# blepping/ComfyUI-sonar

Measured on AMD Instinct MI355X. Metric: noise-latents/sec (SDXL 4x128x128), higher is better.
Workload: dtype f32

## Files before the change

### comfyui-sonar_amd/csrc/plan.hip

```cpp
#include <math.h>
#include <string.h>

#include <memory>
#include <type_traits>
#include <utility>
#include <vector>

#include "common.h"

namespace sonar {
namespace {

template <typename T>
inline T word_to(uint64_t w) {
    if constexpr (std::is_pointer_v<T>) {
        return reinterpret_cast<T>(static_cast<uintptr_t>(w));
    } else if constexpr (std::is_same_v<T, float>) {
        const uint32_t lo = (uint32_t)w;
        float f;
        memcpy(&f, &lo, sizeof f);
        return f;
    } else if constexpr (std::is_same_v<T, double>) {
        double d;
        memcpy(&d, &w, sizeof d);
// ... 42 lines not shown
    SONAR_REPLAYABLE(sonar_philox_normal_chain_f32),
    SONAR_REPLAYABLE(sonar_perlin_lattice_f32),
    SONAR_REPLAYABLE(sonar_perlin_generate_f32),
    SONAR_REPLAYABLE(sonar_perlin_generate_acc_f32),
    SONAR_REPLAYABLE(sonar_perlin_generate_chain_f32),
    SONAR_REPLAYABLE(sonar_perlin_noise_f32),
    SONAR_REPLAYABLE(sonar_perlin_noise_ahead_f32),
    SONAR_REPLAYABLE(sonar_pyramid_generate_f32),
    SONAR_REPLAYABLE(sonar_pyramid_generate_acc_f32),
    SONAR_REPLAYABLE(sonar_pyramid_generate_acc_ahead_f32),
    SONAR_REPLAYABLE(sonar_pyramid_noise_f32),
    SONAR_REPLAYABLE(sonar_pyramid_noise_ahead_f32),
    SONAR_REPLAYABLE(sonar_power_noise_f32),
    SONAR_REPLAYABLE(sonar_power_block_f32),
    SONAR_REPLAYABLE(sonar_power_noise_ahead_f32),
    SONAR_REPLAYABLE(sonar_power_irfft2_f32),
    SONAR_REPLAYABLE(sonar_spectral_filter_f32),
    SONAR_REPLAYABLE(sonar_channel_mix_f32),
    SONAR_REPLAYABLE(sonar_std_scale_f32),
    SONAR_REPLAYABLE(sonar_powerlaw_f32),
    SONAR_REPLAYABLE(sonar_mul_table_f32),
    SONAR_REPLAYABLE(sonar_stats_finalize),
    SONAR_REPLAYABLE(sonar_scale_noise_rows_f32),
    SONAR_REPLAYABLE(sonar_blend_f32),
    SONAR_REPLAYABLE(sonar_blend_tensor_f32),
    SONAR_REPLAYABLE(sonar_scalar_op_f32),
    SONAR_REPLAYABLE(sonar_rowstats_f32),
    SONAR_REPLAYABLE(sonar_row_affine_f32),
    SONAR_REPLAYABLE(sonar_amax_mid_f32),
    SONAR_REPLAYABLE(sonar_div_mid_f32),
// ... 212 lines not shown
```

### comfyui-sonar_amd/csrc/power_fft.hip

```cpp
#include "power_core.h"

namespace sonar {

template <int H, int W>
constexpr int plane_min_waves() {
    return (H * W >= 32768 || (H == 256 && W == 64) || (H == 64 && W == 256) || (H == 64 && W == 32)) ? 2 : 4;
}

template <int H, int W, int SRC, bool STATS, bool NORM>
__global__ void __launch_bounds__((plane_threads<H, W>()), (plane_min_waves<H, W>())) power_irfft2_kernel(const float* __restrict__ z,
                                                                       const float* __restrict__ filter, float* out,
                                                                       int64_t planes, uint64_t seed, uint64_t stream_id,
                                                                       int64_t plane_offset, int group, int split, double* partials,
                                                                       NormArgs na, StatsAhead sa) {
    kernarg_touch_for(z, filter, out, planes, seed, stream_id, plane_offset, group, split, partials, na, sa);
    using C = PlaneCfg<H, W>;
    constexpr int NT = plane_threads<H, W>();
    constexpr int M = C::M, S = C::S;
    constexpr int RN1 = C::RN1, RN2 = C::RN2;
    constexpr bool FAST = (W == 128) && (H == 128 || H == 64) && (NT == 512);
    constexpr int CN1 = FAST ? H / 8 : C::CN1, CN2 = FAST ? 8 : C::CN2;
    __shared__ c32 A[C::kLdsComplex];
    c32* const T0 = A + H * S;
    c32* const TM = T0 + H;
// ... 1021 lines not shown
            }
            partials_next[2 * slot] = ss;
            partials_next[2 * slot + 1] = qq;
        }
    }
};

template <int IT0, int IT1, int N>
__device__ __forceinline__ void pin_chunk(c32 (&v)[N]) {
#pragma unroll
    for (int it = IT0; it < IT1; ++it) {
        asm volatile("" : "+v"(v[it].x), "+v"(v[it].y), "+v"(v[it + N / 2].x), "+v"(v[it + N / 2].y));
    }
}

template <int H, int W, bool STATS, bool NORM>
__global__ void __launch_bounds__(1024) power_pipe_kernel(const float* __restrict__ filter, float* out, int64_t planes, uint64_t seed,
                                                          uint64_t stream_id, int64_t plane_offset, int group, int split, double* partials,
                                                          NormArgs na, uint64_t next_stream, double* partials_next) {
    kernarg_touch_for(filter, out, planes, seed, stream_id, plane_offset, group, split, partials, na, next_stream, partials_next);
    using C = PlaneCfg<H, W>;
    constexpr int NT = 512, NALL = 1024;
    static_assert(plane_threads<H, W>() == NT && W == 128 && H == 128, "one 8-wave team per plane, slot = one radix-16 column item");
    constexpr int M = C::M, S = C::S, Wh = M + 1, RN1 = C::RN1, RN2 = C::RN2, CN1 = H / 8, CN2 = 8, ITER = draw_iters<H, W>();
    constexpr int LM = draw_shift<W>();
    constexpr int E0 = kPipeChunks[0], E1 = E0 + kPipeChunks[1];
    static_assert(E1 <= ITER && ITER == CN1 / 2, "chunks of whole pair iterations");
    constexpr int BUF = H * S;
    __shared__ c32 PLANES[2 * BUF];
    __shared__ c32 EDGE[3 * H];
    __shared__ uint4 SEED_RT[NT];
    static_assert(sizeof(uint4) * NT >= sizeof(c32) * 2 * H * kAheadMaxGroup, "edge columns of a look-ahead unit fit the seed area");
    __shared__ double sred[2 * NT / 64];
    __shared__ double red[2 * NALL / 64];
    __shared__ NormDecision shd;
    const int wv_all = __builtin_amdgcn_readfirstlane((int)threadIdx.x >> 6);
    const bool drawer = wv_all >= NT / 64;
    const int tid = threadIdx.x & (NT - 1), lane = threadIdx.x & 63, wv = wv_all & (NT / 64 - 1);
    const int64_t nunits = split ? planes : planes / group;
    const int64_t group0 = plane_offset / group;
    const int per_unit = split ? 1 : group;
    const int64_t my_units = (int64_t)blockIdx.x < nunits ? (nunits - blockIdx.x + gridDim.x - 1) / gridDim.x : 0;
    const int n = (int)(my_units * per_unit);
    const bool ahead = partials_next != nullptr && nunits <= 2 * (int64_t)gridDim.x;
    const float scale = 1.0f / sqrtf((float)H * (float)W);
    float nm = scale, nc = 0.0f;
    static_assert(!NORM || kNPart == NALL, "one partial pair per thread");
    [[maybe_unused]] double pre_s = 0.0, pre_q = 0.0;
    if constexpr (NORM) {
        pre_s = na.partials[2 * threadIdx.x];
        pre_q = na.partials[2 * threadIdx.x + 1];
    }
    auto leave_wave_sums = [&]() {
        if constexpr (NORM) {
            const double ws = wave_sum(pre_s), wq = wave_sum(pre_q);
            if (lane == 0) {
                red[wv_all] = ws;
                red[NALL / 64 + wv_all] = wq;
            }
        }
    };
    auto decide_in_wave0 = [&]() {
        if constexpr (NORM) {
            if (wv_all == 0) {
                double ss = 0.0, qq = 0.0;
#pragma unroll
                for (int i = 0; i < NALL / 64; ++i) {
                    ss += red[i];
                    qq += red[NALL / 64 + i];
                }
                const NormDecision dec = decision_from_totals(ss, qq, na.n_total, na.thr_sd);
                if (lane == 0) shd = dec;
            }
        }
    };
    auto pick_up_decision = [&]() {
        if constexpr (NORM) {
            const NormDecision dec = shd;
            const float g = (dec.do_div ? 1.0f / dec.stdv : 1.0f) * na.factor;
            nm = scale * g;
            nc = dec.do_sub ? dec.mean * g : 0.0f;
        }
    };
    double s = 0.0, q = 0.0;
    if (drawer) {
        __builtin_amdgcn_s_setprio(kPipePrioDraw);
        const c32* const Q = EDGE + 2 * H;
        SpectrumRng rng;
        float wa[ITER], wb[ITER];
        bool neg = false;
#pragma unroll
        for (int it = 0; it < ITER; ++it) {
            const int p = tid + it * NT, pos = (p >> LM) * Wh + 1 + (p & (M - 1));
            const float fa = filter[pos], fb = filter[pos + (H / 2) * Wh];
            wa[it] = filter_weight(fa);
            wb[it] = filter_weight(fb);
            neg = neg || fa < 0.0f || fb < 0.0f;
        }
        const bool wave_neg = __builtin_amdgcn_ballot_w64(neg) != 0;
        c32 ctw[CN1];
#pragma unroll
        for (int k1 = 0; k1 < CN1; ++k1) ctw[k1] = c_tw256[((wv * k1) * (256 / H)) & 255];
        const int col = (lane + 1) & (M - 1);
        int64_t unit = blockIdx.x;
        int gp = 0;
        for (int j = 0; j < n; ++j) {
            c32* const A = PLANES + (j & 1) * BUF;
            c32 v[CN1];
            SONAR_PIPE_STAMP(0);
            if (gp == 0) {
                const GroupWalk gw(unit, group, split);
                if (j == per_unit) {
                    const uint4 rt = SEED_RT[tid];
                    rng.R = Mwc{rt.x, rt.y};
                    rng.T = Mwc{rt.z, rt.w};
                } else {
                    rng = spectrum_seed<true>(seed, stream_id, group0 + gw.grp, tid, false);
                }
                for (int i = 0; i < gw.first; ++i) skip_plane<H, W, true, false>(rng, tid);
            }
            draw_chunk_regs<H, W, 0, E0>(rng, v, wa, wb);
            if (wave_neg) draw_chunk_signs<H, W, 0, E0>(filter, tid, v);
            pin_chunk<0, E0>(v);
            SONAR_PIPE_STAMP(1);
            __syncthreads();
            draw_chunk_regs<H, W, E0, E1>(rng, v, wa, wb);
            if (wave_neg) draw_chunk_signs<H, W, E0, E1>(filter, tid, v);
            pin_chunk<E0, E1>(v);
            SONAR_PIPE_STAMP(2);
            __syncthreads();
            draw_chunk_regs<H, W, E1, ITER>(rng, v, wa, wb);
            if (wave_neg) draw_chunk_signs<H, W, E1, ITER>(filter, tid, v);
// ... 4 lines not shown
            idft<CN1>(v);
#pragma unroll
            for (int k1 = 1; k1 < CN1; ++k1) v[k1] = cmul(v[k1], ctw[k1]);
#pragma unroll
            for (int k1 = 0; k1 < CN1; ++k1) A[(CN2 * k1 + wv) * S + col] = v[k1];
            if (++gp == per_unit) {
                gp = 0;
                unit += gridDim.x;
            }
            if (j == 0) leave_wave_sums();
            SONAR_PIPE_STAMP(3);
            __syncthreads();
        }
        [[maybe_unused]] const int j = n;
        SONAR_PIPE_STAMP(0);
        if (ahead && my_units == 2) {
            TeamStats<H, W> ts;
            c32* const edge = reinterpret_cast<c32*>(SEED_RT);
            const GroupWalk gw((int64_t)blockIdx.x + gridDim.x, group, split);
            ts.begin(filter, seed, next_stream, plane_offset, group, gw, tid, edge, wa, wb);
            ts.radii(0, kAheadSplitA, tid);
            SONAR_PIPE_STAMP(1);
            __syncthreads();
            ts.radii(kAheadSplitA, kAheadSplitB, tid);
            SONAR_PIPE_STAMP(2);
            __syncthreads();
            ts.radii(kAheadSplitB, 4, tid);
            ts.products();
            ts.edges_and_wave_sums(edge, tid, sred);
            SONAR_PIPE_STAMP(3);
            __syncthreads();
// ... 7 lines not shown
        }
    } else {
        __builtin_amdgcn_s_setprio(kPipePrioFft);
        int64_t unit = blockIdx.x;
        int gp = 0;
        c32* const T0 = EDGE;
        c32* const TM = EDGE + H;
        c32* const Q = EDGE + 2 * H;
        const float f0 = tid < H ? filter[tid * Wh] : 0.0f, fm = tid < H ? filter[tid * Wh + M] : 0.0f;
        Mwc rngE{0, 1}, rngE2{0, 1};
        int64_t eunit = blockIdx.x;
        int egp = 0;
        auto draw_edges = [&](int je) {
            if (tid < H && je < n) {
                if (egp == 0) {
                    const GroupWalk gw(eunit, group, split);
                    rngE = je == per_unit ? rngE2 : spectrum_seed<false>(seed, stream_id, group0 + gw.grp, tid, true).E;
                    for (int i = 0; i < 3 * gw.first; ++i) rngE.next();
                }
                const uint32_t r0 = rngE.next();
                const uint32_t rm = rngE.next();
                const uint32_t t = rngE.next();
                T0[tid] = drawn_elem(r0, angle_lo(t), f0);
                TM[tid] = drawn_elem(rm, angle_hi(t), fm);
                if (++egp == per_unit) {
                    egp = 0;
                    eunit += gridDim.x;
                }
            }
        };
        auto pack_edges = [&](int je) {
            if (tid >= NT - H && je < n) {
                const int ky = tid - (NT - H), kn = (H - ky) & (H - 1);
                const c32 a = T0[ky], an = T0[kn], b = TM[ky], bn = TM[kn];
                Q[ky] = make_float2(0.5f * (a.x + an.x) - 0.5f * (b.y - bn.y), 0.5f * (a.y - an.y) + 0.5f * (b.x + bn.x));
            }
        };
        if (n > per_unit) {
            const GroupWalk gw(unit + gridDim.x, group, split);
            const SpectrumRng g2 = spectrum_rng<H, true>(seed, stream_id, group0 + gw.grp, tid);
            SEED_RT[tid] = make_uint4(g2.R.x, g2.R.c, g2.T.x, g2.T.c);
            rngE2 = g2.E;
        }
        [[maybe_unused]] const int j = 0;
        SONAR_PIPE_STAMP(0);
        auto exchange = [] { __syncthreads(); };
        if (ahead && my_units >= 1) {
            TeamStats<H, W> ts;
            c32* const edge = PLANES + BUF;
            const GroupWalk gw(unit, group, split);
            if (blockIdx.x == 0)
                for (int64_t slot = nunits + tid; slot < kNPart; slot += NT) {
                    partials_next[2 * slot] = 0.0;
                    partials_next[2 * slot + 1] = 0.0;
                }
            __builtin_amdgcn_s_setprio(kAheadPrio);
            draw_edges(0);
            ts.begin(filter, seed, next_stream, plane_offset, group, gw, tid, edge);
            ts.radii(0, kAheadSplitC, tid);
            SONAR_PIPE_STAMP(1);
            exchange();
            pack_edges(0);
// ... 15 lines not shown
            pack_edges(0);
            SONAR_PIPE_STAMP(2);
            exchange();
            leave_wave_sums();
            SONAR_PIPE_STAMP(3);
            __syncthreads();
        }
        for (int j = 1; j <= n; ++j) {
            constexpr int NW = 8;
            const bool work = j >= 1;
            c32* const X = PLANES + ((j + 1) & 1) * BUF;
            c32* const Y = PLANES + (j & 1) * BUF;
            SONAR_PIPE_STAMP(0);
            if (work) pipe_col_b<H, W, NW>(X, Y, wv, lane);
            draw_edges(j);
            if (j == 1) decide_in_wave0();
            SONAR_PIPE_STAMP(1);
            exchange();
            if (work) pipe_row_a<H, W, NW>(Y, X, wv, lane);
            pack_edges(j);
            SONAR_PIPE_STAMP(2);
            exchange();
            if (work) {
                if (j == 1) pick_up_decision();
                const GroupWalk gw(unit, group, split);
                float* const oplane = out + (gw.grp * group + gw.first + gp) * (int64_t)H * W;
                pipe_row_b<H, W, NW, STATS, NORM>(X, oplane, wv, lane, scale, nm, nc, s, q);
                if (++gp == per_unit) {
                    gp = 0;
                    unit += gridDim.x;
                }
            }
            SONAR_PIPE_STAMP(3);
            __syncthreads();
        }
    }
    if (ahead) {
        __syncthreads();
        if (drawer && my_units == 2) TeamStats<H, W>::store(sred, tid, partials_next, (int64_t)blockIdx.x + gridDim.x);
    }
    if constexpr (STATS) write_partial<NALL>(s, q, partials, red);
}

template <int H, int W>
__device__ __forceinline__ void power_stats_body(const float* __restrict__ filter, int64_t planes, uint64_t seed, uint64_t stream_id,
                                                 int64_t plane_offset, int group, int split, double* partials, int64_t bid, int64_t nb,
                                                 c32 (*EDGE)[2][H] , double* red) {
    constexpr int NT = plane_threads<H, W>(), M = W / 2, Wh = M + 1;
    constexpr int NB = kStatsBatch;
    const int tid = threadIdx.x;
    double s = 0.0, q = 0.0;
    auto edge_terms = [&](int p) {
        float edge = 0.0f;
        for (int ky = tid; ky < H; ky += NT) {
            const int kn = (H - ky) & (H - 1);
            const c32 a = EDGE[p][0][ky], an = EDGE[p][0][kn], b = EDGE[p][1][ky], bn = EDGE[p][1][kn];
// ... 352 lines not shown
    SONAR_REQUIRE(filter && out && partials && planes >= 0 && H > 0 && W > 0 && plane_offset >= 0, SONAR_ERR_ARG,
                  "sonar_power_noise_ahead_f32: bad argument");
    SONAR_REQUIRE((reinterpret_cast<uintptr_t>(out) & 7u) == 0 && partials_next != partials, SONAR_ERR_ARG,
                  "sonar_power_noise_ahead_f32: misaligned buffer, or the same workspace for both calls' statistics");
    SONAR_REQUIRE(sonar_power_noise_ahead_ok(planes, H, W, rng_group), SONAR_ERR_UNSUPPORTED,
                  "sonar_power_noise_ahead_f32: no look-ahead for %lld planes of %lld x %lld (ask sonar_power_noise_ahead_ok first)", (long long)planes,
                  (long long)H, (long long)W);
    Ahead ah;
    ah.have_stats = have_stats != 0;
    ah.next_stream = next_stream_id;
    ah.next = partials_next;
    return power_dispatch(1, nullptr, filter, out, planes, H, W, seed, stream_id, plane_offset, rng_group, partials,
                          NormArgs{partials, planes * H * W, factor, threshold_std_devs}, (hipStream_t)stream, ah);
}

extern "C" int sonar_spectral_filter_f32(const float* x, const float* filter, float* out, int64_t planes, int64_t H, int64_t W,
                                         double* partials, void* stream) {
    SONAR_REQUIRE(x && filter && out && x != out && planes >= 0 && H > 0 && W > 0, SONAR_ERR_ARG,
                  "sonar_spectral_filter_f32: bad argument (in-place not supported)");
    SONAR_REQUIRE((reinterpret_cast<uintptr_t>(out) & 7u) == 0 && (reinterpret_cast<uintptr_t>(x) & 7u) == 0, SONAR_ERR_ARG,
                  "sonar_spectral_filter_f32: misaligned buffer");
    if (planes == 0) return SONAR_OK;
    return power_dispatch(3, x, filter, out, planes, H, W, 0, 0, 0, 1, partials, NormArgs{nullptr, 0, 1.0f, 0.0f}, (hipStream_t)stream);
}

extern "C" int sonar_rfft2_f32(const float* x, float* z_out, int64_t planes, int64_t H, int64_t W, void* stream) {
    SONAR_REQUIRE(x && z_out && planes >= 0 && H > 0 && W > 0, SONAR_ERR_ARG, "sonar_rfft2_f32: bad argument");
    SONAR_REQUIRE((reinterpret_cast<uintptr_t>(z_out) & 7u) == 0 && (reinterpret_cast<uintptr_t>(x) & 7u) == 0, SONAR_ERR_ARG,
                  "sonar_rfft2_f32: misaligned buffer");
    if (planes == 0) return SONAR_OK;
// ... 27 lines not shown
```

### comfyui-sonar_amd/hip_lib.py

```python
from __future__ import annotations

import ctypes as C
import math
import os
import threading as _threading
import weakref
from typing import Optional, Sequence

import torch

_HERE = os.path.dirname(os.path.abspath(__file__))
LIB_PATH = os.path.join(_HERE, "libsonar_hip.so")

BLEND_IDS = {"lerp": 0, "inject": 1, "subtract_b": 2}
MODE_IDS = {"CLASSIC": 0, "NEW": 1, "DENOISED": 2}
INIT_IDS = {"NONE": 0, "SAMPLE": 1, "SAMPLE_NORM": 2}
RESAMPLE_IDS = {"bilinear": 0, "nearest-exact": 1, "area": 2, "adaptive_avg_pool2d": 2, "nearest": 3, "bicubic": 4, "bicubic_aligned": 5,
                "bilinear_aligned": 6}
UPSCALE_MODES = ("bilinear", "nearest-exact", "area", "adaptive_avg_pool2d", "nearest", "bicubic")
PYRAMID_FUSED_MODES = ("bilinear", "nearest-exact", "area", "adaptive_avg_pool2d")
DWT_MODE_IDS = {"zero": 0, "symmetric": 1, "reflect": 2, "periodization": 3, "periodic": 4, "constant": 5, "replicate": 5}
NPART = 1024
BROWNIAN_MAX_TERMS = 96
ERR_ARG, ERR_UNSUPPORTED, ERR_HIP = -1, -2, -3
# ... 93 lines not shown
    "sonar_perlin_noise_ahead_ok": (_I, [_I64, _I64, _I64]),
    "sonar_perlin_noise_ahead_f32": (_I, [_P, _P, _I64, _I64, _F, _U64, _U64, _I64, _F, _F, _P, _I, _U64, _P, _P, _P, _I64, _I64, _I64, _I64, _I, _U64, _P]),
    "sonar_resample_acc_f32": (_I, [_P, _P, _I64, _I64, _I64, _I64, _I64, _F, _I, _I, _P, _P]),
    "sonar_pyramid_generate_f32": (_I, [_P, _I64, _I64, _I64, _I64, C.POINTER(_P), _PI64, _PI64, _PF, _I, _U64, _U64, _I64, _P, _P]),
    "sonar_pyramid_route": (_I, [_I64, _I64, _I64, _PI64, _PI64, _I, _I64]),
    "sonar_pyramid_noise_f32": (_I, [_P, _I64, _I64, _I64, _I64, C.POINTER(_P), _PI64, _PI64, _PF, _I, _U64, _U64, _I64, _F, _F, _P, _P]),
    "sonar_pyramid_noise_ahead_f32": (_I, [_P, _I64, _I64, _I64, _I64, _PI64, _PI64, _PF, _I, _U64, _U64, _I64, _F, _F, _P, _I, _U64, _I64, _PI64, _PI64, _PF, _P,
                                           _P]),
    "sonar_levels_sampled_f32": (_I, [_P, _I64, _I64, _I64, _I, _PI64, _PI64, _PF, _PF, _I, _U64, _U64, _I64, _I, _P]),
    "sonar_level_normal_f32": (_I, [_P, _I64, _I64, _I64, _F, _U64, _U64, _I64, _P]),
    "sonar_power_noise_f32": (_I, [_P, _P, _I64, _I64, _I64, _U64, _U64, _I64, _I, _F, _F, _P, _P]),
    "sonar_power_noise_ahead_ok": (_I, [_I64, _I64, _I64, _I]),
    "sonar_power_pipeline": (_I, [_I]),
    "sonar_wcfg_hi_storage": (_I, [_I]),
    "sonar_power_noise_ahead_f32": (_I, [_P, _P, _I64, _I64, _I64, _U64, _U64, _I64, _I, _F, _F, _P, _I, _U64, _P, _P]),
    "sonar_power_spectrum_f32": (_I, [_P, _I64, _I64, _I64, _U64, _U64, _I64, _I, _P]),
    "sonar_power_irfft2_f32": (_I, [_P, _P, _P, _I64, _I64, _I64, _U64, _U64, _I64, _I, _P, _P]),
    "sonar_spectral_filter_f32": (_I, [_P, _P, _P, _I64, _I64, _I64, _P, _P]),
    "sonar_std_scale_f32": (_I, [_P, _I64, _F, _P, _I64, _I64, _P]),
    "sonar_channel_mix_f32": (_I, [_P, _P, _P, _I64, _I64, _I64, _P, _P]),
    "sonar_dwt_out_len": (_I64, [_I64, _I64, _I]),
    "sonar_dwt2_ws_bytes": (_I64, [_I64, _I64, _I64, _I, _I, _I, _I]),
    "sonar_dwt2_fwd_f32": (_I, [_P, _P, _P, _I64, _I64, _I64, _PD, _PD, _I, _I, _P, _P]),
    "sonar_dwt2_fwd_f64": (_I, [_P, _P, _P, _I64, _I64, _I64, _PD, _PD, _I, _I, _P, _P]),
    "sonar_dwt2_inv_f32": (_I, [_P, _I64, _I64, _P, _P, _I64, _I64, _I64, _I64, _I64, _PD, _PD, _I, _I, _P, _P]),
    "sonar_dwt2_inv_f64": (_I, [_P, _I64, _I64, _P, _P, _I64, _I64, _I64, _I64, _I64, _PD, _PD, _I, _I, _P, _P]),
    "sonar_sq_acc_f32": (_I, [_P, _P, _F, _I, _I64, _P]),
    "sonar_studentt_f32": (_I, [_P, _P, _F, _F, _F, _I64, _P]),
    "sonar_abs_quantile_rows_f32": (_I, [_P, _I64, _I64, _I64, _F, _P, _P]),
    "sonar_clamp_signpow_rows_f32": (_I, [_P, _I64, _I64, _P, _F, _F, _P]),
# ... 992 lines not shown
    if kind in (3, 4):
        if z is None:
            white = philox_normal(tuple(shape), filt.device, seed, stream_id, plane_offset * H * W)
            return _direct_spectral_filter(white, filt, partials)
        return _direct_inverse(z, filt, out, 1.0 / math.sqrt(H * W), partials)
    _check(
        load().sonar_power_irfft2_f32(zp, _dev(filt, "filter"), _dev(out, "out"), planes, H, W, seed & (2**64 - 1), stream_id, plane_offset,
                                      rng_group_for(shape), _opt(partials, "partials", torch.float64), _stream()),
        "sonar_power_irfft2_f32",
    )
    return out


class PowerLookahead:

    __slots__ = ("key", "partials", "last_stream", "last_delta", "step", "hits", "misses")

    def __init__(self):
        self.key = None
        self.partials = None
        self.last_stream = None
        self.last_delta = None
        self.step = 1
        self.hits = 0
        self.misses = 0


def power_noise(filt: torch.Tensor, shape, *, seed: int, stream_id: int, plane_offset: int, factor: float,
                threshold_std_devs: float = 2.5, lookahead: Optional[PowerLookahead] = None) -> torch.Tensor:
    H, W = shape[-2:]
    out = torch.empty(shape, dtype=torch.float32, device=filt.device)
    planes = out.numel() // (H * W)
    kind = power_plane_kind(H, W)
    if kind == 4:
        return _power_block(1, filt, out, seed, stream_id, plane_offset, partials=new_partials(filt.device), factor=factor,
                            threshold_std_devs=threshold_std_devs)
    if kind == 3:
        ws = new_partials(filt.device)
        white = philox_normal(tuple(shape), filt.device, seed, stream_id, plane_offset * H * W)
        return scale_noise_(_direct_spectral_filter(white, filt, ws), factor, True, ws, threshold_std_devs=threshold_std_devs)
    group = rng_group_for(shape)
    lib = load()
    seed &= 2**64 - 1
    if lookahead is not None and lib.sonar_power_noise_ahead_ok(planes, H, W, group):
        st = _stream()

        def key_for(stream, seed=seed, st=st):
            return (filt.data_ptr(), filt._version, tuple(shape), seed, stream, plane_offset, group, filt.device, st)

        have = lookahead.key is not None and lookahead.key == key_for(stream_id)
        ws = lookahead.partials if have else new_partials(filt.device)
        if lookahead.last_stream is not None and stream_id > lookahead.last_stream:
            delta = stream_id - lookahead.last_stream
            if lookahead.last_delta is None or delta == lookahead.last_delta:
                lookahead.step = delta
            lookahead.last_delta = delta
        nxt = (stream_id + lookahead.step) & (2**64 - 1)
        nws = new_partials(filt.device)
        _check(
            lib.sonar_power_noise_ahead_f32(_dev(filt, "filter"), _dev(out, "out"), planes, H, W, seed, stream_id, plane_offset, group,
                                            float(factor), float(threshold_std_devs), _dev(ws, "ws", torch.float64), int(have), nxt,
                                            _dev(nws, "ws_next", torch.float64), st),
            "sonar_power_noise_ahead_f32",
        )
        lookahead.hits += int(have)
        lookahead.misses += int(not have)
        lookahead.key, lookahead.partials, lookahead.last_stream = key_for(nxt), nws, stream_id
        rec = _recorder
        if rec is not None and rec.thread == _threading.get_ident():
            if have and lookahead.last_delta == lookahead.step:
                rec.hooks.append(_PowerAheadHook(lookahead, key_for, ws, nws, stream_id - rec.base, lookahead.step, filt.device))
            else:
                rec.fail("power-law look-ahead not in its steady state")
        return out
    ws = new_partials(filt.device)
    _check(
        lib.sonar_power_noise_f32(_dev(filt, "filter"), _dev(out, "out"), planes, H, W, seed, stream_id, plane_offset,
                                  group, float(factor), float(threshold_std_devs), _dev(ws, "ws", torch.float64), _stream()),
        "sonar_power_noise_f32",
    )
    return out


# ... 861 lines not shown
        return out


def wcfg_fused(cond: torch.Tensor, uncond: torch.Tensor, x: Optional[torch.Tensor], **params):
    return FusedCall(**params)(cond, uncond, x)


PLANS_ENABLED = os.environ.get("SONAR_PLANS", "1") != "0"
PLAN_WARM_CALLS = 2
PLAN_MAX_ATTEMPTS = 3
FILL_AHEAD = os.environ.get("SONAR_FILL_AHEAD", "1") != "0"
PYRAMID_AHEAD = os.environ.get("SONAR_PYRAMID_AHEAD", "1") != "0"
PERLIN_AHEAD = os.environ.get("SONAR_PERLIN_AHEAD", "1") != "0"
NOT_RUN = object()
_M64 = 2**64 - 1
_HOST_QUERIES = frozenset(("sonar_abi_version", "sonar_noise_stream_version", "sonar_last_error", "sonar_noise_params_ws_doubles", "sonar_group_stats_ws_doubles", "sonar_power_noise_ahead_ok", "sonar_perlin_noise_ahead_ok", "sonar_philox_noise_ahead_ok", "sonar_power_pipeline", "sonar_wcfg_hi_storage", "sonar_power_plane_kind", "sonar_power_any_plan", "sonar_dwt_out_len",
                           "sonar_dwt2_ws_bytes", "sonar_wcfg_lowpass_lds_bytes", "sonar_wcfg_fused_ws_bytes", "sonar_pyramid_levels", "sonar_pyramid_route",
                           "sonar_plan_fn_id", "sonar_plan_fn_nargs"))
PATCH_SLOT, PATCH_STREAM, PATCH_SEED, PATCH_BLOB, PATCH_LEVELS = range(5)


class PlanPatch(C.Structure):

    _fields_ = [("source", C.c_int32), ("target", C.c_int32), ("index", C.c_int32), ("width", C.c_int32), ("addend", C.c_int64)]


class PlanLevels(C.Structure):

    _fields_ = [("H", C.c_int64), ("W", C.c_int64), ("discount", C.c_double), ("iterations", C.c_int32), ("reserved", C.c_int32),
                ("h_offset", C.c_int64), ("w_offset", C.c_int64), ("weight_offset", C.c_int64)]

# ... 832 lines not shown
```

### comfyui-sonar_amd/py/nodes/powernoise.py

```python
from __future__ import annotations

import importlib
import math
import os
import random
import tempfile

import torch
from torch import Tensor

from ... import hip_lib
from ..noise import CustomNoiseItemBase
from ..noise_generation import BrownianTreeNoiseSampler, DeviceRNG, current_batch_offset
from .. import utils
from ..utils import attach_stats, pop_stats, scale_noise


def _host_module(name: str):
    try:
        return importlib.import_module(name)
    except ModuleNotFoundError as exc:
        if exc.name is not None and (name == exc.name or name.startswith(exc.name + ".")):
            return None
        raise
# ... 168 lines not shown
        filt = filt.to(device, torch.float32).reshape(1, 1, h, w // 2 + 1).contiguous()
        ones = torch.ones((1, 1, h, w // 2 + 1), dtype=torch.complex64, device=device)
        return filt, hip_lib.power_irfft2(ones, filt, (1, 1, h, w))


def _device_irfft2_fallback_error(h, w):
    return hip_lib.SonarHipError(
        f"power noise: plane {h}x{w} is beyond the spectral kernels (LDS-resident FFTs, direct passes up to 2048 x 2048); "
        "there is no CPU fallback"
    )


class PowerNoiseItem(CustomNoiseItemBase):

    stats_lookahead = True

    def __init__(self, factor, *, channel_correlation, power_filter=None, **kwargs):
        if isinstance(channel_correlation, str):
            vals = tuple(float(v) for v in (v.strip() for v in channel_correlation.split(",")) if v)
            channel_correlation = torch.tensor(vals, device="cpu", dtype=torch.float)
        if power_filter is None:
            fargs = {k: kwargs.pop(k) for k in ("min_freq", "max_freq", "stretch", "rotate", "pnorm", "alpha") if k in kwargs}
            power_filter = PowerFilter(**fargs)
        super().__init__(factor, power_filter=power_filter, channel_correlation=channel_correlation, **kwargs)

    def make_filter(self, shape, oversample=None):
        with utils.host_setup_threads():
            return PowerFilter.normalize(self.power_filter.build(shape, override_oversample=oversample), shape, mix=self.mix,
                                         normalization_factor=getattr(self, "filter_norm_factor", 1.0))

    def make_noise_sampler_internal(self, x: Tensor, noise_sampler, filter_rfft, normalized=True):
        shape = tuple(x.shape)
        h, w = shape[-2:]
        if x.ndim < 4:
            raise hip_lib.SonarHipError("power noise: [B, C, ..., H, W] latents (4 or more dimensions)")
        if not hip_lib.power_supported(h, w):
            raise _device_irfft2_fallback_error(h, w)
        device = x.device
        filt = filter_rfft.to(device, torch.float32).reshape(h, w // 2 + 1).contiguous()
        with utils.host_setup_threads():
            mixer = ChannelMixer(shape[1], self.common_mode, self.channel_correlation)
            identity = mixer.is_identity
        mixer.to(device)
        planes_per_latent = math.prod(shape[1:-2])
        lookahead = hip_lib.PowerLookahead() if self.stats_lookahead else None

        def sampler(sigma, sigma_next):
            z = noise_sampler(sigma, sigma_next)
            partials = hip_lib.new_partials(device)
            if self.time_brownian:
                pop_stats(z)
                noise = hip_lib.spectral_filter(z.to(device).contiguous(), filt, partials if (identity and normalized) else None)
            elif z is None:
                seed, stream = DeviceRNG.take()
                offs = current_batch_offset() * planes_per_latent
                if identity and normalized:
                    return hip_lib.power_noise(filt, shape, seed=seed, stream_id=stream, plane_offset=offs, factor=self.factor,
                                               lookahead=lookahead)
                noise = hip_lib.power_irfft2(None, filt, shape, seed=seed, stream_id=stream, plane_offset=offs,
                                             partials=partials if (identity and normalized) else None)
# ... 103 lines not shown
```

### include/sonar_hip.h

```cpp
#ifndef SONAR_HIP_H
#define SONAR_HIP_H

#include <stdint.h>

#ifdef __cplusplus
extern "C" {
#endif

#define SONAR_OK 0
#define SONAR_ERR_ARG (-1)
#define SONAR_ERR_UNSUPPORTED (-2)
#define SONAR_ERR_HIP (-3)

#define SONAR_BLEND_LERP 0
#define SONAR_BLEND_INJECT 1
#define SONAR_BLEND_SUBTRACT_B 2

#define SONAR_MODE_CLASSIC 0
#define SONAR_MODE_NEW 1
#define SONAR_MODE_DENOISED 2

#define SONAR_INIT_NONE 0
#define SONAR_INIT_SAMPLE 1
#define SONAR_INIT_SAMPLE_NORM 2
// ... 403 lines not shown
int sonar_power_block_f32(const float* filter, float* ws, float* out, int64_t planes, int64_t H, int64_t W, uint64_t seed, uint64_t stream_id,
                          int64_t plane_offset, int rng_group, int mode, float factor, float threshold_std_devs, double* partials ,
                          void* stream);
int sonar_power_irfft2_f32(const float* z, const float* filter, float* out, int64_t planes, int64_t H, int64_t W,
                           uint64_t seed, uint64_t stream_id, int64_t plane_offset, int rng_group,
                           double* partials , void* stream);
int sonar_power_noise_f32(const float* filter, float* out, int64_t planes, int64_t H, int64_t W, uint64_t seed,
                          uint64_t stream_id, int64_t plane_offset, int rng_group, float factor, float threshold_std_devs,
                          double* partials , void* stream);

int sonar_power_noise_ahead_ok(int64_t planes, int64_t H, int64_t W, int rng_group);
int sonar_power_pipeline(int enable);
int sonar_power_noise_ahead_f32(const float* filter, float* out, int64_t planes, int64_t H, int64_t W, uint64_t seed,
                                uint64_t stream_id, int64_t plane_offset, int rng_group, float factor, float threshold_std_devs,
                                double* partials, int have_stats, uint64_t next_stream_id, double* partials_next, void* stream);
int sonar_power_spectrum_f32(float* z_out, int64_t planes, int64_t H, int64_t W, uint64_t seed, uint64_t stream_id,
                             int64_t plane_offset, int rng_group, void* stream);
int sonar_spectral_filter_f32(const float* x, const float* filter, float* out, int64_t planes, int64_t H, int64_t W,
                              double* partials, void* stream);
int sonar_std_scale_f32(float* x, int64_t n, float mul, const double* partials, int64_t npart, int64_t n_total, void* stream);
int sonar_channel_mix_f32(const float* in, const float* mixer, float* out, int64_t B, int64_t C, int64_t hw,
                          double* partials , void* stream);

int64_t sonar_dwt_out_len(int64_t n, int64_t flen, int mode);
int64_t sonar_dwt2_ws_bytes(int64_t planes, int64_t H, int64_t W, int flen, int mode, int elem_size, int inverse);
int sonar_dwt2_fwd_f32(const float* x, float* ll, float* hi, int64_t planes, int64_t H, int64_t W,
                       const double* dec_lo, const double* dec_hi, int flen, int mode, void* ws, void* stream);
int sonar_dwt2_fwd_f64(const double* x, double* ll, double* hi, int64_t planes, int64_t H, int64_t W,
                       const double* dec_lo, const double* dec_hi, int flen, int mode, void* ws, void* stream);
int sonar_dwt2_inv_f32(const float* ll, int64_t ll_h, int64_t ll_w, const float* hi, float* out, int64_t planes,
// ... 110 lines not shown
```

Measured before the change: 12.61 million.

## Draw two consecutive power-noise steps per launch and hold the second

Adds a pair variant of the pipelined power-noise kernel. One launch generates the normalised noise for the current stream and for the next step's stream, and computes look-ahead statistics for the two steps after that. The Python lookahead keeps the second output and returns it on the next call when its key matches, so most steps cost one launch per two calls and the grid holds twice as many units. In exchange it uses more LDS and a held output buffer per lookahead, and it only applies to 128x128 planes with more than 256 planes, outside Brownian-time mode. It also stops the graph recorder from capturing this path.

```diff
diff --git a/comfyui-sonar_amd/csrc/plan.hip b/comfyui-sonar_amd/csrc/plan.hip
--- a/comfyui-sonar_amd/csrc/plan.hip
+++ b/comfyui-sonar_amd/csrc/plan.hip
@@ -80,6 +80,7 @@
     SONAR_REPLAYABLE(sonar_power_noise_f32),
     SONAR_REPLAYABLE(sonar_power_block_f32),
     SONAR_REPLAYABLE(sonar_power_noise_ahead_f32),
+    SONAR_REPLAYABLE(sonar_power_noise_pair_f32),
     SONAR_REPLAYABLE(sonar_power_irfft2_f32),
     SONAR_REPLAYABLE(sonar_spectral_filter_f32),
     SONAR_REPLAYABLE(sonar_channel_mix_f32),
diff --git a/comfyui-sonar_amd/csrc/power_fft.hip b/comfyui-sonar_amd/csrc/power_fft.hip
--- a/comfyui-sonar_amd/csrc/power_fft.hip
+++ b/comfyui-sonar_amd/csrc/power_fft.hip
@@ -1059,11 +1059,19 @@
     }
 }
 
-template <int H, int W, bool STATS, bool NORM>
-__global__ void __launch_bounds__(1024) power_pipe_kernel(const float* __restrict__ filter, float* out, int64_t planes, uint64_t seed,
-                                                          uint64_t stream_id, int64_t plane_offset, int group, int split, double* partials,
-                                                          NormArgs na, uint64_t next_stream, double* partials_next) {
-    kernarg_touch_for(filter, out, planes, seed, stream_id, plane_offset, group, split, partials, na, next_stream, partials_next);
+struct PairArgs {
+    float* out_b = nullptr;
+    uint64_t stream_b = 0;
+    const double* partials_b = nullptr;
+    uint64_t next2_stream = 0;
+    double* partials_next2 = nullptr;
+};
+
+template <int H, int W, bool STATS, bool NORM, bool PAIR>
+__device__ __forceinline__ void power_pipe_body(const float* __restrict__ filter, float* out, int64_t planes, uint64_t seed, uint64_t stream_id,
+                                                int64_t plane_offset, int group, int split, double* partials, NormArgs na,
+                                                uint64_t next_stream, double* partials_next, const PairArgs& pa) {
+    static_assert(!PAIR || (NORM && !STATS), "the pair form is the normalised generate call's");
     using C = PlaneCfg<H, W>;
     constexpr int NT = 512, NALL = 1024;
     static_assert(plane_threads<H, W>() == NT && W == 128 && H == 128, "one 8-wave team per plane, slot = one radix-16 column item");
@@ -1076,25 +1084,44 @@
     __shared__ c32 EDGE[3 * H];
     __shared__ uint4 SEED_RT[NT];
     static_assert(sizeof(uint4) * NT >= sizeof(c32) * 2 * H * kAheadMaxGroup, "edge columns of a look-ahead unit fit the seed area");
-    __shared__ double sred[2 * NT / 64];
-    __shared__ double red[2 * NALL / 64];
+    constexpr int SR = 2 * NT / 64;
+    __shared__ c32 EDGE2[PAIR ? 2 * H * kAheadMaxGroup : 1];
+    __shared__ double sred[(PAIR ? 4 : 1) * SR];
+    __shared__ double red[(PAIR ? 2 : 1) * 2 * NALL / 64];
     __shared__ NormDecision shd;
+    __shared__ NormDecision shd_b;
     const int wv_all = __builtin_amdgcn_readfirstlane((int)threadIdx.x >> 6);
     const bool drawer = wv_all >= NT / 64;
     const int tid = threadIdx.x & (NT - 1), lane = threadIdx.x & 63, wv = wv_all & (NT / 64 - 1);
     const int64_t nunits = split ? planes : planes / group;
     const int64_t group0 = plane_offset / group;
     const int per_unit = split ? 1 : group;
-    const int64_t my_units = (int64_t)blockIdx.x < nunits ? (nunits - blockIdx.x + gridDim.x - 1) / gridDim.x : 0;
+    const int64_t tunits = PAIR ? 2 * nunits : nunits;
+    const int64_t my_units = (int64_t)blockIdx.x < tunits ? (tunits - blockIdx.x + gridDim.x - 1) / gridDim.x : 0;
+    auto in_b = [&](int64_t u) -> bool {
+        if constexpr (PAIR) return u >= nunits;
+        return false;
+    };
+    auto local_unit = [&](int64_t u) -> int64_t { return in_b(u) ? u - nunits : u; };
+    auto stream_of = [&](int64_t u) -> uint64_t {
+        if constexpr (PAIR) return u >= nunits ? pa.stream_b : stream_id;
+        return stream_id;
+    };
     const int n = (int)(my_units * per_unit);
     const bool ahead = partials_next != nullptr && nunits <= 2 * (int64_t)gridDim.x;
     const float scale = 1.0f / sqrtf((float)H * (float)W);
     float nm = scale, nc = 0.0f;
+    [[maybe_unused]] float nm_b = scale, nc_b = 0.0f;
     static_assert(!NORM || kNPart == NALL, "one partial pair per thread");
     [[maybe_unused]] double pre_s = 0.0, pre_q = 0.0;
     if constexpr (NORM) {
         pre_s = na.partials[2 * threadIdx.x];
         pre_q = na.partials[2 * threadIdx.x + 1];
+    }
+    [[maybe_unused]] double pre_sb = 0.0, pre_qb = 0.0;
+    if constexpr (PAIR) {
+        pre_sb = pa.partials_b[2 * threadIdx.x];
+        pre_qb = pa.partials_b[2 * threadIdx.x + 1];
     }
     auto leave_wave_sums = [&]() {
         if constexpr (NORM) {
@@ -1104,27 +1131,50 @@
                 red[NALL / 64 + wv_all] = wq;
             }
         }
+        if constexpr (PAIR) {
+            const double ws = wave_sum(pre_sb), wq = wave_sum(pre_qb);
+            if (lane == 0) {
+                red[2 * NALL / 64 + wv_all] = ws;
+                red[3 * NALL / 64 + wv_all] = wq;
+            }
+        }
     };
-    auto decide_in_wave0 = [&]() {
+    auto decide_in_wave0 = [&](int j) {
         if constexpr (NORM) {
-            if (wv_all == 0) {
+            if (wv_all == 0 && (j == 1 || (PAIR && j == 2))) {
+                const double* const r = red + (j == 2 ? 2 * NALL / 64 : 0);
                 double ss = 0.0, qq = 0.0;
 #pragma unroll
                 for (int i = 0; i < NALL / 64; ++i) {
-                    ss += red[i];
-                    qq += red[NALL / 64 + i];
+                    ss += r[i];
+                    qq += r[NALL / 64 + i];
                 }
                 const NormDecision dec = decision_from_totals(ss, qq, na.n_total, na.thr_sd);
-                if (lane == 0) shd = dec;
+                if (lane == 0) {
+                    if (j == 1) shd = dec;
+                    else shd_b = dec;
+                }
             }
         }
     };
-    auto pick_up_decision = [&]() {
+    auto pick_up_decision = [&](int j) {
         if constexpr (NORM) {
-            const NormDecision dec = shd;
-            const float g = (dec.do_div ? 1.0f / dec.stdv : 1.0f) * na.factor;
-            nm = scale * g;
-            nc = dec.do_sub ? dec.mean * g : 0.0f;
+            if constexpr (!PAIR) {
+                if (j == 1) {
+                    const NormDecision dec = shd;
+                    const float g = (dec.do_div ? 1.0f / dec.stdv : 1.0f) * na.factor;
+                    nm = scale * g;
+                    nc = dec.do_sub ? dec.mean * g : 0.0f;
+                }
+            } else if (j == 1 || j == 2) {
+                const NormDecision dec = j == 1 ? shd : shd_b;
+                const float g = (dec.do_div ? 1.0f / dec.stdv : 1.0f) * na.factor;
+                const float m = scale * g, c = dec.do_sub ? dec.mean * g : 0.0f;
+                nm = j == 1 ? m : nm;
+                nc = j == 1 ? c : nc;
+                nm_b = j == 2 ? m : nm_b;
+                nc_b = j == 2 ? c : nc_b;
+            }
         }
     };
     double s = 0.0, q = 0.0;
@@ -1154,13 +1204,13 @@
             c32 v[CN1];
             SONAR_PIPE_STAMP(0);
             if (gp == 0) {
-                const GroupWalk gw(unit, group, split);
+                const GroupWalk gw(local_unit(unit), group, split);
                 if (j == per_unit) {
                     const uint4 rt = SEED_RT[tid];
                     rng.R = Mwc{rt.x, rt.y};
                     rng.T = Mwc{rt.z, rt.w};
                 } else {
-                    rng = spectrum_seed<true>(seed, stream_id, group0 + gw.grp, tid, false);
+                    rng = spectrum_seed<true>(seed, stream_of(unit), group0 + gw.grp, tid, false);
                 }
                 for (int i = 0; i < gw.first; ++i) skip_plane<H, W, true, false>(rng, tid);
             }
@@ -1195,7 +1245,32 @@
         }
         [[maybe_unused]] const int j = n;
         SONAR_PIPE_STAMP(0);
-        if (ahead && my_units == 2) {
+        if constexpr (PAIR) {
+            TeamStats<H, W> ts1, ts2;
+            c32* const edge = reinterpret_cast<c32*>(SEED_RT);
+            const int64_t u1 = blockIdx.x, u2 = u1 + gridDim.x;
+            const bool two = u2 < nunits;
+            ts1.begin(filter, seed, pa.next2_stream, plane_offset, group, GroupWalk(u1, group, split), tid, edge, wa, wb);
+            ts1.radii(0, 2, tid);
+            SONAR_PIPE_STAMP(1);
+            __syncthreads();
+            ts1.radii(2, 4, tid);
+            ts1.products();
+            ts1.edges_and_wave_sums(edge, tid, sred + 2 * SR);
+            if (two) {
+                ts2.begin(filter, seed, pa.next2_stream, plane_offset, group, GroupWalk(u2, group, split), tid, EDGE2, wa, wb);
+                ts2.radii(0, 2, tid);
+            }
+            SONAR_PIPE_STAMP(2);
+            __syncthreads();
+            if (two) {
+                ts2.radii(2, 4, tid);
+                ts2.products();
+                ts2.edges_and_wave_sums(EDGE2, tid, sred + 3 * SR);
+            }
+            SONAR_PIPE_STAMP(3);
+            __syncthreads();
+        } else if (ahead && my_units == 2) {
             TeamStats<H, W> ts;
             c32* const edge = reinterpret_cast<c32*>(SEED_RT);
             const GroupWalk gw((int64_t)blockIdx.x + gridDim.x, group, split);
@@ -1233,8 +1308,8 @@
         auto draw_edges = [&](int je) {
             if (tid < H && je < n) {
                 if (egp == 0) {
-                    const GroupWalk gw(eunit, group, split);
-                    rngE = je == per_unit ? rngE2 : spectrum_seed<false>(seed, stream_id, group0 + gw.grp, tid, true).E;
+                    const GroupWalk gw(local_unit(eunit), group, split);
+                    rngE = je == per_unit ? rngE2 : spectrum_seed<false>(seed, stream_of(eunit), group0 + gw.grp, tid, true).E;
                     for (int i = 0; i < 3 * gw.first; ++i) rngE.next();
                 }
                 const uint32_t r0 = rngE.next();
@@ -1256,15 +1331,55 @@
             }
         };
         if (n > per_unit) {
-            const GroupWalk gw(unit + gridDim.x, group, split);
-            const SpectrumRng g2 = spectrum_rng<H, true>(seed, stream_id, group0 + gw.grp, tid);
+            const GroupWalk gw(local_unit(unit + gridDim.x), group, split);
+            const SpectrumRng g2 = spectrum_rng<H, true>(seed, stream_of(unit + gridDim.x), group0 + gw.grp, tid);
             SEED_RT[tid] = make_uint4(g2.R.x, g2.R.c, g2.T.x, g2.T.c);
             rngE2 = g2.E;
         }
         [[maybe_unused]] const int j = 0;
         SONAR_PIPE_STAMP(0);
         auto exchange = [] { __syncthreads(); };
-        if (ahead && my_units >= 1) {
+        if constexpr (PAIR) {
+            TeamStats<H, W> ts1, ts2;
+            c32* const edge1 = PLANES + BUF;
+            c32* const edge2 = edge1 + 2 * H * kAheadMaxGroup;
+            static_assert(2 * 2 * H * kAheadMaxGroup <= BUF, "two look-ahead units' edge columns fit a plane buffer");
+            const int64_t u1 = blockIdx.x, u2 = u1 + gridDim.x;
+            const bool two = u2 < nunits;
+            if (blockIdx.x == 0)
+                for (int64_t slot = nunits + tid; slot < kNPart; slot += NT) {
+                    partials_next[2 * slot] = 0.0;
+                    partials_next[2 * slot + 1] = 0.0;
+                    pa.partials_next2[2 * slot] = 0.0;
+                    pa.partials_next2[2 * slot + 1] = 0.0;
+                }
+            __builtin_amdgcn_s_setprio(kAheadPrio);
+            draw_edges(0);
+            ts1.begin(filter, seed, next_stream, plane_offset, group, GroupWalk(u1, group, split), tid, edge1);
+            ts1.radii(0, 4, tid);
+            ts1.products();
+            SONAR_PIPE_STAMP(1);
+            exchange();
+            pack_edges(0);
+            ts1.edges_and_wave_sums(edge1, tid, sred);
+            if (two) {
+                ts2.begin(filter, seed, next_stream, plane_offset, group, GroupWalk(u2, group, split), tid, edge2);
+                ts2.radii(0, 2, tid);
+            }
+            SONAR_PIPE_STAMP(2);
+            exchange();
+            if (two) {
+                ts2.radii(2, 4, tid);
+                ts2.products();
+                ts2.edges_and_wave_sums(edge2, tid, sred + SR);
+            }
+            leave_wave_sums();
+            SONAR_PIPE_STAMP(3);
+            __syncthreads();
+            TeamStats<H, W>::store(sred, tid, partials_next, u1);
+            if (two) TeamStats<H, W>::store(sred + SR, tid, partials_next, u2);
+            __builtin_amdgcn_s_setprio(kPipePrioFft);
+        } else if (ahead && my_units >= 1) {
             TeamStats<H, W> ts;
             c32* const edge = PLANES + BUF;
             const GroupWalk gw(unit, group, split);
@@ -1310,7 +1425,7 @@
             SONAR_PIPE_STAMP(0);
             if (work) pipe_col_b<H, W, NW>(X, Y, wv, lane);
             draw_edges(j);
-            if (j == 1) decide_in_wave0();
+            decide_in_wave0(j);
             SONAR_PIPE_STAMP(1);
             exchange();
             if (work) pipe_row_a<H, W, NW>(Y, X, wv, lane);
@@ -1318,10 +1433,11 @@
             SONAR_PIPE_STAMP(2);
             exchange();
             if (work) {
-                if (j == 1) pick_up_decision();
-                const GroupWalk gw(unit, group, split);
-                float* const oplane = out + (gw.grp * group + gw.first + gp) * (int64_t)H * W;
-                pipe_row_b<H, W, NW, STATS, NORM>(X, oplane, wv, lane, scale, nm, nc, s, q);
+                pick_up_decision(j);
+                const GroupWalk gw(local_unit(unit), group, split);
+                const bool ub = in_b(unit);
+                float* const oplane = (ub ? pa.out_b : out) + (gw.grp * group + gw.first + gp) * (int64_t)H * W;
+                pipe_row_b<H, W, NW, STATS, NORM>(X, oplane, wv, lane, scale, ub ? nm_b : nm, ub ? nc_b : nc, s, q);
                 if (++gp == per_unit) {
                     gp = 0;
                     unit += gridDim.x;
@@ -1331,11 +1447,35 @@
             __syncthreads();
         }
     }
-    if (ahead) {
+    if constexpr (PAIR) {
+        __syncthreads();
+        if (drawer) {
+            TeamStats<H, W>::store(sred + 2 * SR, tid, pa.partials_next2, (int64_t)blockIdx.x);
+            if ((int64_t)blockIdx.x + gridDim.x < nunits) TeamStats<H, W>::store(sred + 3 * SR, tid, pa.partials_next2, (int64_t)blockIdx.x + gridDim.x);
+        }
+    } else if (ahead) {
         __syncthreads();
         if (drawer && my_units == 2) TeamStats<H, W>::store(sred, tid, partials_next, (int64_t)blockIdx.x + gridDim.x);
     }
     if constexpr (STATS) write_partial<NALL>(s, q, partials, red);
+}
+
+template <int H, int W, bool STATS, bool NORM>
+__global__ void __launch_bounds__(1024) power_pipe_kernel(const float* __restrict__ filter, float* out, int64_t planes, uint64_t seed,
+                                                          uint64_t stream_id, int64_t plane_offset, int group, int split, double* partials,
+                                                          NormArgs na, uint64_t next_stream, double* partials_next) {
+    kernarg_touch_for(filter, out, planes, seed, stream_id, plane_offset, group, split, partials, na, next_stream, partials_next);
+    power_pipe_body<H, W, STATS, NORM, false>(filter, out, planes, seed, stream_id, plane_offset, group, split, partials, na, next_stream, partials_next,
+                                              PairArgs());
+}
+
+template <int H, int W>
+__global__ void __launch_bounds__(1024) power_pipe_pair_kernel(const float* __restrict__ filter, float* out, int64_t planes, uint64_t seed,
+                                                               uint64_t stream_id, int64_t plane_offset, int group, int split, NormArgs na,
+                                                               uint64_t next_stream, double* partials_next, PairArgs pa) {
+    kernarg_touch_for(filter, out, planes, seed, stream_id, plane_offset, group, split, na, next_stream, partials_next, pa);
+    power_pipe_body<H, W, false, true, true>(filter, out, planes, seed, stream_id, plane_offset, group, split, (double*)nullptr, na, next_stream,
+                                             partials_next, pa);
 }
 
 template <int H, int W>
@@ -1718,6 +1858,52 @@
                           NormArgs{partials, planes * H * W, factor, threshold_std_devs}, (hipStream_t)stream, ah);
 }
 
+extern "C" int sonar_power_noise_pair_ok(int64_t planes, int64_t H, int64_t W, int rng_group) {
+    if (H != 128 || W != 128 || !pipe_enabled() || planes <= 256) return 0;
+    return sonar_power_noise_ahead_ok(planes, H, W, rng_group);
+}
+
+extern "C" int sonar_power_noise_pair_f32(const float* filter, float* out_a, float* out_b, int64_t planes, int64_t H, int64_t W, uint64_t seed,
+                                          uint64_t stream_a, uint64_t stream_b, int64_t plane_offset, int rng_group, float factor,
+                                          float threshold_std_devs, double* partials_a, int have_a, double* partials_b, int have_b,
+                                          uint64_t next1_stream_id, double* partials_next1, uint64_t next2_stream_id, double* partials_next2,
+                                          void* stream) {
+    SONAR_REQUIRE(filter && out_a && out_b && partials_a && partials_b && partials_next1 && partials_next2 && planes >= 0 && H > 0 && W > 0 &&
+                      plane_offset >= 0,
+                  SONAR_ERR_ARG, "sonar_power_noise_pair_f32: bad argument");
+    const uintptr_t oa = reinterpret_cast<uintptr_t>(out_a), ob = reinterpret_cast<uintptr_t>(out_b);
+    const uintptr_t obytes = (uintptr_t)planes * (uintptr_t)H * (uintptr_t)W * sizeof(float);
+    SONAR_REQUIRE((oa & 7u) == 0 && (ob & 7u) == 0 && (oa + obytes <= ob || ob + obytes <= oa), SONAR_ERR_ARG,
+                  "sonar_power_noise_pair_f32: misaligned buffer, or the two calls' outputs overlap");
+    SONAR_REQUIRE(partials_a != partials_b && partials_a != partials_next1 && partials_a != partials_next2 && partials_b != partials_next1 &&
+                      partials_b != partials_next2 && partials_next1 != partials_next2,
+                  SONAR_ERR_ARG, "sonar_power_noise_pair_f32: the same workspace for two calls' statistics");
+    SONAR_REQUIRE(rng_group >= 1 && rng_group <= kMaxRngGroup && planes % rng_group == 0 && plane_offset % rng_group == 0, SONAR_ERR_ARG,
+                  "sonar_power_noise_pair_f32: planes (%lld) and plane_offset (%lld) must be multiples of the RNG group (%d, at most %d)",
+                  (long long)planes, (long long)plane_offset, rng_group, kMaxRngGroup);
+    SONAR_REQUIRE(sonar_power_noise_pair_ok(planes, H, W, rng_group), SONAR_ERR_UNSUPPORTED,
+                  "sonar_power_noise_pair_f32: no pair launch for %lld planes of %lld x %lld (ask sonar_power_noise_pair_ok first)", (long long)planes,
+                  (long long)H, (long long)W);
+    const hipStream_t st = (hipStream_t)stream;
+    int psplit;
+    const int64_t units = pipe_units(planes, rng_group, &psplit);
+    const int pg = (int)std::min<int64_t>(units, 256);
+    const dim3 sgrid(std::min<int64_t>(units, kNPart)), sblk(plane_threads<128, 128>());
+    if (!have_a)
+        hipLaunchKernelGGL((power_stats_kernel<128, 128>), sgrid, sblk, 0, st, filter, planes, seed, stream_a, plane_offset, rng_group, psplit, partials_a);
+    if (!have_b)
+        hipLaunchKernelGGL((power_stats_kernel<128, 128>), sgrid, sblk, 0, st, filter, planes, seed, stream_b, plane_offset, rng_group, psplit, partials_b);
+    PairArgs pa;
+    pa.out_b = out_b;
+    pa.stream_b = stream_b;
+    pa.partials_b = partials_b;
+    pa.next2_stream = next2_stream_id;
+    pa.partials_next2 = partials_next2;
+    hipLaunchKernelGGL((power_pipe_pair_kernel<128, 128>), dim3(pg), dim3(1024), 0, st, filter, out_a, planes, seed, stream_a, plane_offset, rng_group, psplit,
+                       NormArgs{partials_a, planes * H * W, factor, threshold_std_devs}, next1_stream_id, partials_next1, pa);
+    return check_launch("sonar_power_noise_pair_f32");
+}
+
 extern "C" int sonar_spectral_filter_f32(const float* x, const float* filter, float* out, int64_t planes, int64_t H, int64_t W,
                                          double* partials, void* stream) {
     SONAR_REQUIRE(x && filter && out && x != out && planes >= 0 && H > 0 && W > 0, SONAR_ERR_ARG,
diff --git a/comfyui-sonar_amd/hip_lib.py b/comfyui-sonar_amd/hip_lib.py
--- a/comfyui-sonar_amd/hip_lib.py
+++ b/comfyui-sonar_amd/hip_lib.py
@@ -131,6 +131,8 @@
     "sonar_power_pipeline": (_I, [_I]),
     "sonar_wcfg_hi_storage": (_I, [_I]),
     "sonar_power_noise_ahead_f32": (_I, [_P, _P, _I64, _I64, _I64, _U64, _U64, _I64, _I, _F, _F, _P, _I, _U64, _P, _P]),
+    "sonar_power_noise_pair_ok": (_I, [_I64, _I64, _I64, _I]),
+    "sonar_power_noise_pair_f32": (_I, [_P, _P, _P, _I64, _I64, _I64, _U64, _U64, _U64, _I64, _I, _F, _F, _P, _I, _P, _I, _U64, _P, _U64, _P, _P]),
     "sonar_power_spectrum_f32": (_I, [_P, _I64, _I64, _I64, _U64, _U64, _I64, _I, _P]),
     "sonar_power_irfft2_f32": (_I, [_P, _P, _P, _I64, _I64, _I64, _U64, _U64, _I64, _I, _P, _P]),
     "sonar_spectral_filter_f32": (_I, [_P, _P, _P, _I64, _I64, _I64, _P, _P]),
@@ -1153,9 +1155,17 @@
 
 class PowerLookahead:
 
-    __slots__ = ("key", "partials", "last_stream", "last_delta", "step", "hits", "misses")
-
-    def __init__(self):
+    __slots__ = ("key", "partials", "last_stream", "last_delta", "step", "hits", "misses", "draw_ahead", "held", "held_key", "key2", "partials2",
+                 "pairs")
+    DRAW_AHEAD_MAX_BYTES = 256 << 20
+
+    def __init__(self, draw_ahead: bool = False):
+        self.draw_ahead = bool(draw_ahead)
+        self.held = None
+        self.held_key = None
+        self.key2 = None
+        self.partials2 = None
+        self.pairs = 0
         self.key = None
         self.partials = None
         self.last_stream = None
@@ -1168,6 +1178,19 @@
 def power_noise(filt: torch.Tensor, shape, *, seed: int, stream_id: int, plane_offset: int, factor: float,
                 threshold_std_devs: float = 2.5, lookahead: Optional[PowerLookahead] = None) -> torch.Tensor:
     H, W = shape[-2:]
+    rec = _recorder
+    if lookahead is not None and lookahead.held_key is not None:
+        seed_m = seed & (2**64 - 1)
+        held, held_key = lookahead.held, lookahead.held_key
+        lookahead.held = lookahead.held_key = None
+        if held_key == (filt.data_ptr(), filt._version, tuple(shape), seed_m, stream_id, plane_offset, rng_group_for(shape), filt.device, _stream()):
+            lookahead.hits += 1
+            lookahead.last_delta, lookahead.last_stream = stream_id - lookahead.last_stream, stream_id
+            if rec is not None and rec.thread == _threading.get_ident():
+                rec.fail("power-law draw-ahead: the step is one launch per two calls")
+            return held
+        del held
+        lookahead.key = lookahead.partials = lookahead.key2 = lookahead.partials2 = None
     out = torch.empty(shape, dtype=torch.float32, device=filt.device)
     planes = out.numel() // (H * W)
     kind = power_plane_kind(H, W)
@@ -1195,6 +1218,30 @@
                 lookahead.step = delta
             lookahead.last_delta = delta
         nxt = (stream_id + lookahead.step) & (2**64 - 1)
+        if (lookahead.draw_ahead and out.numel() * 4 <= lookahead.DRAW_AHEAD_MAX_BYTES
+                and lib.sonar_power_noise_pair_ok(planes, H, W, group)):
+            step = lookahead.step
+            nxt1, nxt2 = (stream_id + 2 * step) & (2**64 - 1), (stream_id + 3 * step) & (2**64 - 1)
+            have_b = have and lookahead.key2 is not None and lookahead.key2 == key_for(nxt)
+            ws_b = lookahead.partials2 if have_b else new_partials(filt.device)
+            out_b = torch.empty(shape, dtype=torch.float32, device=filt.device)
+            nws, nws2 = new_partials(filt.device), new_partials(filt.device)
+            _check(
+                lib.sonar_power_noise_pair_f32(_dev(filt, "filter"), _dev(out, "out"), _dev(out_b, "out_next"), planes, H, W, seed, stream_id, nxt,
+                                               plane_offset, group, float(factor), float(threshold_std_devs), _dev(ws, "ws", torch.float64),
+                                               int(have), _dev(ws_b, "ws_next", torch.float64), int(have_b), nxt1,
+                                               _dev(nws, "ws_next1", torch.float64), nxt2, _dev(nws2, "ws_next2", torch.float64), st),
+                "sonar_power_noise_pair_f32",
+            )
+            lookahead.hits += int(have)
+            lookahead.misses += int(not have)
+            lookahead.pairs += 1
+            lookahead.held, lookahead.held_key = out_b, key_for(nxt)
+            lookahead.key, lookahead.partials, lookahead.last_stream = key_for(nxt1), nws, stream_id
+            lookahead.key2, lookahead.partials2 = key_for(nxt2), nws2
+            if rec is not None and rec.thread == _threading.get_ident():
+                rec.fail("power-law draw-ahead: the step is one launch per two calls")
+            return out
         nws = new_partials(filt.device)
         _check(
             lib.sonar_power_noise_ahead_f32(_dev(filt, "filter"), _dev(out, "out"), planes, H, W, seed, stream_id, plane_offset, group,
@@ -1205,7 +1252,6 @@
         lookahead.hits += int(have)
         lookahead.misses += int(not have)
         lookahead.key, lookahead.partials, lookahead.last_stream = key_for(nxt), nws, stream_id
-        rec = _recorder
         if rec is not None and rec.thread == _threading.get_ident():
             if have and lookahead.last_delta == lookahead.step:
                 rec.hooks.append(_PowerAheadHook(lookahead, key_for, ws, nws, stream_id - rec.base, lookahead.step, filt.device))
@@ -2097,7 +2143,7 @@
 PERLIN_AHEAD = os.environ.get("SONAR_PERLIN_AHEAD", "1") != "0"
 NOT_RUN = object()
 _M64 = 2**64 - 1
-_HOST_QUERIES = frozenset(("sonar_abi_version", "sonar_noise_stream_version", "sonar_last_error", "sonar_noise_params_ws_doubles", "sonar_group_stats_ws_doubles", "sonar_power_noise_ahead_ok", "sonar_perlin_noise_ahead_ok", "sonar_philox_noise_ahead_ok", "sonar_power_pipeline", "sonar_wcfg_hi_storage", "sonar_power_plane_kind", "sonar_power_any_plan", "sonar_dwt_out_len",
+_HOST_QUERIES = frozenset(("sonar_abi_version", "sonar_noise_stream_version", "sonar_last_error", "sonar_noise_params_ws_doubles", "sonar_group_stats_ws_doubles", "sonar_power_noise_ahead_ok", "sonar_power_noise_pair_ok", "sonar_perlin_noise_ahead_ok", "sonar_philox_noise_ahead_ok", "sonar_power_pipeline", "sonar_wcfg_hi_storage", "sonar_power_plane_kind", "sonar_power_any_plan", "sonar_dwt_out_len",
                            "sonar_dwt2_ws_bytes", "sonar_wcfg_lowpass_lds_bytes", "sonar_wcfg_fused_ws_bytes", "sonar_pyramid_levels", "sonar_pyramid_route",
                            "sonar_plan_fn_id", "sonar_plan_fn_nargs"))
 PATCH_SLOT, PATCH_STREAM, PATCH_SEED, PATCH_BLOB, PATCH_LEVELS = range(5)
diff --git a/comfyui-sonar_amd/py/nodes/powernoise.py b/comfyui-sonar_amd/py/nodes/powernoise.py
--- a/comfyui-sonar_amd/py/nodes/powernoise.py
+++ b/comfyui-sonar_amd/py/nodes/powernoise.py
@@ -206,6 +206,7 @@
 class PowerNoiseItem(CustomNoiseItemBase):
 
     stats_lookahead = True
+    draw_ahead = True
 
     def __init__(self, factor, *, channel_correlation, power_filter=None, **kwargs):
         if isinstance(channel_correlation, str):
@@ -236,6 +237,8 @@
         mixer.to(device)
         planes_per_latent = math.prod(shape[1:-2])
         lookahead = hip_lib.PowerLookahead() if self.stats_lookahead else None
+        if lookahead is not None:
+            lookahead.draw_ahead = bool(self.draw_ahead) and not self.time_brownian
 
         def sampler(sigma, sigma_next):
             z = noise_sampler(sigma, sigma_next)
diff --git a/include/sonar_hip.h b/include/sonar_hip.h
--- a/include/sonar_hip.h
+++ b/include/sonar_hip.h
@@ -441,6 +441,12 @@
 int sonar_power_noise_ahead_f32(const float* filter, float* out, int64_t planes, int64_t H, int64_t W, uint64_t seed,
                                 uint64_t stream_id, int64_t plane_offset, int rng_group, float factor, float threshold_std_devs,
                                 double* partials, int have_stats, uint64_t next_stream_id, double* partials_next, void* stream);
+int sonar_power_noise_pair_ok(int64_t planes, int64_t H, int64_t W, int rng_group);
+int sonar_power_noise_pair_f32(const float* filter, float* out_a, float* out_b, int64_t planes, int64_t H, int64_t W, uint64_t seed,
+                               uint64_t stream_a, uint64_t stream_b, int64_t plane_offset, int rng_group, float factor,
+                               float threshold_std_devs, double* partials_a, int have_a, double* partials_b, int have_b,
+                               uint64_t next1_stream_id, double* partials_next1, uint64_t next2_stream_id, double* partials_next2,
+                               void* stream);
 int sonar_power_spectrum_f32(float* z_out, int64_t planes, int64_t H, int64_t W, uint64_t seed, uint64_t stream_id,
                              int64_t plane_offset, int rng_group, void* stream);
 int sonar_spectral_filter_f32(const float* x, const float* filter, float* out, int64_t planes, int64_t H, int64_t W,
```

After: 12.43 million. -1.4%, worse.
